# howardlau1999/pytorch-ddp-template

Hardware: NVIDIA H100
Metric: samples/sec (whole box, device-timed, max over ranks) for ResNet-50 DDP at 1/2/4/8 H100 (higher is better)
Workload: dtype bf16; 1 GPU; model=resnet50, global_batch=32, per_gpu_batch=32, image_size=224, parallelism=dp1, loss=mse(dense one-hot target), optimizer=sgd lr1e-3 + clip_grad_norm 1000 + linear warmup/decay, transport=single, cuda_graph=True

## Files before the change

b200ddp/csrc/batchnorm.cu:

```cuda
#include "ops.h"
#include "drv.h"
#include "tc_primitives.cuh"

#include <algorithm>
#include <cstdlib>
#include <map>
#include <mutex>
#include <utility>

namespace b200 {
namespace {

constexpr int kBnThreads = 256;
constexpr int kVec = 8;

template <typename T> __device__ __forceinline__ void bn_load8(const T* p, float* f);
template <> __device__ __forceinline__ void bn_load8<__nv_bfloat16>(const __nv_bfloat16* p, float* f) {
  unpack8(*reinterpret_cast<const Bf16x8*>(p), f);
}
template <> __device__ __forceinline__ void bn_load8<float>(const float* p, float* f) {
  const float4 a = reinterpret_cast<const float4*>(p)[0], b = reinterpret_cast<const float4*>(p)[1];
  f[0] = a.x; f[1] = a.y; f[2] = a.z; f[3] = a.w; f[4] = b.x; f[5] = b.y; f[6] = b.z; f[7] = b.w;
}
template <typename T> __device__ __forceinline__ void bn_store8(T* p, const float* f);
// ... 439 lines not shown
  const int cv = blockIdx.x * cvb + tx;
  if (cv * kVec >= C) return;
  const int S = gridDim.y;
  const int rows_per = (R + S - 1) / S;
  const int r0 = blockIdx.y * rows_per, r1 = min(R, r0 + rows_per);
  bn_bwd_apply_rows<T>(dy, x, y, dx, dres, save_mean, save_rstd, gamma, coef, C, cv, r0, r1, tyi, ty, relu);
}

template <typename T>
__global__ void __launch_bounds__(kBnThreads) bn_bwd_apply_pdl_kernel(const T* __restrict__ dy, const T* __restrict__ x, const unsigned char* __restrict__ y,
                                                                     T* __restrict__ dx, T* __restrict__ dres, const float* __restrict__ save_mean,
                                                                     const float* __restrict__ save_rstd, const float* __restrict__ gamma,
                                                                     const float* __restrict__ coef, int R, int C, int cvb, int ty, int relu) {
  const int tx = threadIdx.x % cvb, tyi = threadIdx.x / cvb;
  const int cv = blockIdx.x * cvb + tx;
  const int S = gridDim.y;
  const int rows_per = (R + S - 1) / S;
  const int r0 = blockIdx.y * rows_per, r1 = min(R, r0 + rows_per);
  bn_wait_producer();
  if (cv * kVec >= C) return;
  bn_bwd_apply_rows<T>(dy, x, y, dx, dres, save_mean, save_rstd, gamma, coef, C, cv, r0, r1, tyi, ty, relu);
}

int g_bn_pdl = -1;
bool bn_pdl_enabled() {
  if (g_bn_pdl < 0) { const char* e = getenv("B200DDP_PDL"); g_bn_pdl = (e && atoi(e) != 0) ? 1 : 0; }
  return g_bn_pdl > 0;
}

template <typename... KArgs, typename... Args>
void launch_dependent(void (*kernel)(KArgs...), dim3 grid, cudaStream_t s, Args... args) {
  cudaLaunchConfig_t cfg = {};
  cfg.gridDim = grid;
  cfg.blockDim = dim3(kBnThreads);
  cfg.dynamicSmemBytes = 0;
  cfg.stream = s;
  cudaLaunchAttribute attr[1];
  attr[0].id = cudaLaunchAttributeProgrammaticStreamSerialization;
  attr[0].val.programmaticStreamSerializationAllowed = 1;
  cfg.attrs = attr;
  cfg.numAttrs = 1;
  B200_CUDA_CHECK(cudaLaunchKernelEx(&cfg, kernel, static_cast<KArgs>(args)...));
}

Tile pick_tile(int R, int C) {
  Tile t;
  const int cv = C / kVec;
  t.cvb = cv < 8 ? cv : 8;
  while (kBnThreads % t.cvb != 0) --t.cvb;
  t.ty = kBnThreads / t.cvb;
  t.grid_x = (cv + t.cvb - 1) / t.cvb;
  int want = (4 * kNumSMs + t.grid_x - 1) / t.grid_x;
  int max_by_rows = R / (t.ty * 4);
  if (max_by_rows < 1) max_by_rows = 1;
  t.grid_y = want < max_by_rows ? want : max_by_rows;
  if (t.grid_y > 256) t.grid_y = 256;
  return t;
}

dim3 apply_grid(const Tile& t, int R) {
  int want = (8 * kNumSMs + t.grid_x - 1) / t.grid_x;
  int max_by_rows = R / (t.ty * 4);
  if (max_by_rows < 1) max_by_rows = 1;
  int gy = want < max_by_rows ? want : max_by_rows;
  return dim3(t.grid_x, gy);
}

bool fused_tile(int R, int C, Tile* t) {
  static int enabled = -1;
  if (enabled < 0) { const char* e = getenv("B200DDP_BN_FUSED"); enabled = (e && atoi(e) == 1) ? 1 : 0; }
  *t = pick_tile(R, C);
  if (!enabled || t->grid_x > 2 * kNumSMs) return false;
  int cap = (2 * kNumSMs) / t->grid_x;
  if (cap < 1) cap = 1;
  if (t->grid_y > cap) t->grid_y = cap;
  return true;
}

constexpr int kResThreads = 256;
constexpr int kResTile = 64;
constexpr int kResMaxBox = 256;
constexpr int kResMaxBoxes = 16;
constexpr int kResWarps = kResThreads / 32;
constexpr int kResMaxWaves = 2;
constexpr int kResFixedSmem = kResMaxBoxes * 8 + (kResWarps * 2 + 2 + 3) * kResTile * 4;

__device__ unsigned int g_bn_resident_error = 0;

struct ResGeom {
  int R, C;
  int T;
  int P;
  int box_rows;
  int nbox;
  int waves;
};

__device__ __forceinline__ void res_grid_sync(unsigned int* bar, unsigned int nblocks) {
  __syncthreads();
  if (threadIdx.x == 0) {
    unsigned int* gen = bar + 1;
    const unsigned int g0 = bn_ld_acquire(gen);
    __threadfence();
    if (atomicAdd(bar, 1u) == nblocks - 1) {
      atomicExch(bar, 0u);
      __threadfence();
      bn_st_release(gen, g0 + 1u);
    } else {
      unsigned long long t0;
      asm volatile("mov.u64 %0, %%globaltimer;" : "=l"(t0));
      while (bn_ld_acquire(gen) == g0) {
        unsigned long long t;
        asm volatile("mov.u64 %0, %%globaltimer;" : "=l"(t));
        if (t - t0 > 2000000000ull) { atomicExch(&g_bn_resident_error, 1u); break; }
      }
    }
    __threadfence();
  }
  __syncthreads();
}

__device__ __forceinline__ void res_write_partials(float (&acc)[2][kVec], float* red, float* __restrict__ partial, int P, int p, int C,
                                                   int c0) {
  const int lane = threadIdx.x & 31, warp = threadIdx.x >> 5, cv = threadIdx.x & 7;
#pragma unroll
  for (int a = 0; a < 2; ++a)
#pragma unroll
    for (int i = 0; i < kVec; ++i) {
      float v = acc[a][i];
      v += __shfl_xor_sync(0xffffffffu, v, 8);
      v += __shfl_xor_sync(0xffffffffu, v, 16);
      if (lane < 8) red[(warp * 2 + a) * kResTile + cv * kVec + i] = v;
    }
  __syncthreads();
  if (threadIdx.x < 2 * kResTile) {
    const int a = threadIdx.x / kResTile, c = threadIdx.x % kResTile;
    float s = 0.f;
    for (int w = 0; w < kResWarps; ++w) s += red[(w * 2 + a) * kResTile + c];
    if (c0 + c < C) partial[((size_t)a * P + p) * C + c0 + c] = s;
  }
}

__device__ __forceinline__ void res_reduce_partials(float* red, const float* __restrict__ partial, int P, int C, int c0) {
  const int q = threadIdx.x & 31, l = threadIdx.x >> 5;
  const int a = q >> 4, c4 = (q & 15) * 4;
  float4 s = make_float4(0.f, 0.f, 0.f, 0.f);
  if (c0 + c4 < C) {
    const float* base = partial + (size_t)a * P * C + c0 + c4;
#pragma unroll 4
    for (int k = l; k < P; k += kResWarps) {
      const float4 v = __ldcg(reinterpret_cast<const float4*>(base + (size_t)k * C));
      s.x += v.x; s.y += v.y; s.z += v.z; s.w += v.w;
    }
  }
  __syncthreads();
  *reinterpret_cast<float4*>(red + (l * 2 + a) * kResTile + c4) = s;
  __syncthreads();
  if (threadIdx.x < 2 * kResTile) {
    const int aa = threadIdx.x / kResTile, c = threadIdx.x % kResTile;
    float t = 0.f;
    for (int w = 0; w < kResWarps; ++w) t += red[(w * 2 + aa) * kResTile + c];
    red[kResWarps * 2 * kResTile + aa * kResTile + c] = t;
  }
  __syncthreads();
}

__device__ __forceinline__ void res_ld8(const unsigned char* s, float* f) { unpack8(*reinterpret_cast<const Bf16x8*>(s), f); }
__device__ __forceinline__ void res_st8(unsigned char* s, const float* f) { *reinterpret_cast<Bf16x8*>(s) = pack8(f); }

__global__ void __launch_bounds__(kResThreads, 2)
bn_resident_fwd_kernel(const __grid_constant__ CUtensorMap map_x, const __grid_constant__ CUtensorMap map_y,
                       const __grid_constant__ CUtensorMap map_res, const __nv_bfloat16* __restrict__ residual, unsigned char* __restrict__ mask, const float* __restrict__ gamma,
                       const float* __restrict__ beta, float* __restrict__ running_mean, float* __restrict__ running_var,
                       long long* __restrict__ num_batches, float* __restrict__ save_mean, float* __restrict__ save_rstd,
                       float* __restrict__ scale, float* __restrict__ shift, float* __restrict__ partial, unsigned int* __restrict__ bar,
                       float eps, float momentum, int relu, const ResGeom g) {
  extern __shared__ __align__(128) unsigned char res_smem[];
  const int slab_rows = g.nbox * g.box_rows;
  const uint32_t box_bytes = (uint32_t)g.box_rows * kResTile * 2;
  unsigned char* data = res_smem;
  uint64_t* mbar = reinterpret_cast<uint64_t*>(res_smem + (size_t)slab_rows * kResTile * 2);
  float* red = reinterpret_cast<float*>(mbar + kResMaxBoxes);
  float* coef = red + kResWarps * 2 * kResTile + 2 * kResTile;
  const int cv = threadIdx.x & 7, rl = threadIdx.x >> 3;
  const int ntiles = (g.C + kResTile - 1) / kResTile, cvs = g.C / kVec;
  const int slot = blockIdx.x / g.P, p = blockIdx.x % g.P;
  const int r0 = p * slab_rows;
  const int nlive = r0 >= g.R ? 0 : min(g.nbox, (g.R - r0 + g.box_rows - 1) / g.box_rows);
  if (threadIdx.x == 0) {
    for (int b = 0; b < g.nbox; ++b) tc::mbar_init(&mbar[b], 1);
    asm volatile("fence.mbarrier_init.release.cluster;" ::: "memory");
    tc::tma_prefetch_desc(&map_x);
    tc::tma_prefetch_desc(&map_y);
    if (blockIdx.x == 0 && num_batches != nullptr) *num_batches += 1;
  }
  __syncthreads();
  for (int w = 0; w < g.waves; ++w) {
    const int t = w * g.T + slot;
    const bool active = t < ntiles;
    const int c0 = t * kResTile;
    const int cvg = t * (kResTile / kVec) + cv;
    if (active && threadIdx.x == 0) {
      for (int b = 0; b < nlive; ++b) {
        tc::mbar_expect_tx(&mbar[b], box_bytes);
        tc::tma_load_2d(&map_x, &mbar[b], data + (size_t)b * box_bytes, c0, r0 + b * g.box_rows);
      }
    }
    float acc[2][kVec];
#pragma unroll
    for (int i = 0; i < kVec; ++i) { acc[0][i] = 0.f; acc[1][i] = 0.f; }
    if (active) {
      for (int b = 0; b < nlive; ++b) {
        tc::mbar_wait(&mbar[b], (uint32_t)(w & 1));
        const unsigned char* box = data + (size_t)b * box_bytes + cv * 16;
        for (int rr = rl; rr < g.box_rows; rr += 4 * 32) {
          float f[4][kVec];
#pragma unroll
          for (int u = 0; u < 4; ++u) {
            if (rr + u * 32 < g.box_rows) res_ld8(box + (size_t)(rr + u * 32) * (kResTile * 2), f[u]);
            else
#pragma unroll
              for (int i = 0; i < kVec; ++i) f[u][i] = 0.f;
          }
#pragma unroll
          for (int u = 0; u < 4; ++u)
#pragma unroll
            for (int i = 0; i < kVec; ++i) { acc[0][i] += f[u][i]; acc[1][i] = fmaf(f[u][i], f[u][i], acc[1][i]); }
        }
      }
      if (residual != nullptr && threadIdx.x == 0) {
        for (int b = 0; b < nlive; ++b)
          asm volatile("cp.async.bulk.prefetch.tensor.2d.L2.global [%0, {%1, %2}];"
                       ::"l"(reinterpret_cast<uint64_t>(&map_res)), "r"(c0), "r"(r0 + b * g.box_rows) : "memory");
      }
      res_write_partials(acc, red, partial, g.P, p, g.C, c0);
    }
    res_grid_sync(bar, gridDim.x);
    if (!active) continue;
    res_reduce_partials(red, partial, g.P, g.C, c0);
    if (threadIdx.x < kResTile) {
      const float* tot = red + kResWarps * 2 * kResTile;
      const int c = threadIdx.x, ch = c0 + c;
      if (ch < g.C) {
        const float inv_r = 1.f / (float)g.R;
        const float mean = tot[c] * inv_r;
        const float var = fmaxf(tot[kResTile + c] * inv_r - mean * mean, 0.f);
        const float rstd = rsqrtf(var + eps);
        const float sc = gamma[ch] * rstd;
        const float sh = beta[ch] - mean * sc;
        coef[c] = sc;
        coef[kResTile + c] = sh;
        if (p == 0) {
          save_mean[ch] = mean;
          save_rstd[ch] = rstd;
          scale[ch] = sc;
          shift[ch] = sh;
          if (running_mean != nullptr) {
            const float unbiased = g.R > 1 ? var * ((float)g.R / (float)(g.R - 1)) : var;
            running_mean[ch] = (1.f - momentum) * running_mean[ch] + momentum * mean;
            running_var[ch] = (1.f - momentum) * running_var[ch] + momentum * unbiased;
          }
        }
      } else {
        coef[c] = 0.f;
        coef[kResTile + c] = 0.f;
      }
    }
    __syncthreads();
    float sc[kVec], sh[kVec];
#pragma unroll
    for (int i = 0; i < kVec; ++i) { sc[i] = coef[cv * kVec + i]; sh[i] = coef[kResTile + cv * kVec + i]; }
    const bool live_cv = cvg < cvs;
    for (int b = 0; b < nlive; ++b) {
      unsigned char* box = data + (size_t)b * box_bytes + cv * 16;
      const int rb = r0 + b * g.box_rows;
      for (int rr = rl; rr < g.box_rows; rr += 8 * 32) {
        Bf16x8 rv[8];
#pragma unroll
        for (int u = 0; u < 8; ++u) {
          const int r = rb + rr + u * 32;
          if (residual != nullptr && rr + u * 32 < g.box_rows && r < g.R && live_cv)
            rv[u] = *reinterpret_cast<const Bf16x8*>(residual + (size_t)r * g.C + (size_t)cvg * kVec);
        }
#pragma unroll
        for (int u = 0; u < 8; ++u) {
          const int r = rb + rr + u * 32;
          if (!(rr + u * 32 < g.box_rows && r < g.R && live_cv)) continue;
          float f[kVec], rs[kVec];
          res_ld8(box + (size_t)(rr + u * 32) * (kResTile * 2), f);
          if (residual != nullptr) unpack8(rv[u], rs);
          unsigned int bits = 0;
#pragma unroll
          for (int i = 0; i < kVec; ++i) {
            float v = fmaf(f[i], sc[i], sh[i]);
            if (residual != nullptr) v += rs[i];
            bits |= (v > 0.f ? 1u : 0u) << i;
            f[i] = relu ? fmaxf(v, 0.f) : v;
          }
          res_st8(box + (size_t)(rr + u * 32) * (kResTile * 2), f);
          if (mask != nullptr) mask[(size_t)r * cvs + cvg] = (unsigned char)bits;
        }
      }
      tc::fence_async_smem();
      __syncthreads();
      if (threadIdx.x == 0) { tc::tma_store_2d(&map_y, data + (size_t)b * box_bytes, c0, rb); tc::bulk_commit(); }
    }
    if (threadIdx.x == 0) asm volatile("cp.async.bulk.wait_group.read 0;" ::: "memory");
    __syncthreads();
  }
  if (threadIdx.x == 0) tc::bulk_wait_all();
}

__global__ void __launch_bounds__(kResThreads, 2)
bn_resident_bwd_kernel(const __grid_constant__ CUtensorMap map_dy, const __grid_constant__ CUtensorMap map_x,
                       const __grid_constant__ CUtensorMap map_dx, const __grid_constant__ CUtensorMap map_dres,
                       const unsigned char* __restrict__ mask, const float* __restrict__ save_mean, const float* __restrict__ save_rstd,
                       const float* __restrict__ gamma, float* __restrict__ dgamma, float* __restrict__ dbeta, float* __restrict__ coef_out,
                       float* __restrict__ partial, unsigned int* __restrict__ bar, int relu, int want_dres, const ResGeom g) {
  extern __shared__ __align__(128) unsigned char res_smem[];
  const int slab_rows = g.nbox * g.box_rows;
  const uint32_t box_bytes = (uint32_t)g.box_rows * kResTile * 2;
  unsigned char* dyd = res_smem;
  unsigned char* xd = res_smem + (size_t)slab_rows * kResTile * 2;
  uint64_t* mbar = reinterpret_cast<uint64_t*>(res_smem + (size_t)2 * slab_rows * kResTile * 2);
  float* red = reinterpret_cast<float*>(mbar + kResMaxBoxes);
  float* coef = red + kResWarps * 2 * kResTile + 2 * kResTile;
  unsigned char* smask = reinterpret_cast<unsigned char*>(coef + 3 * kResTile);
  const int cv = threadIdx.x & 7, rl = threadIdx.x >> 3;
  const int ntiles = (g.C + kResTile - 1) / kResTile, cvs = g.C / kVec;
  const int slot = blockIdx.x / g.P, p = blockIdx.x % g.P;
  const int r0 = p * slab_rows;
  const int nlive = r0 >= g.R ? 0 : min(g.nbox, (g.R - r0 + g.box_rows - 1) / g.box_rows);
  if (threadIdx.x == 0) {
    for (int b = 0; b < g.nbox; ++b) tc::mbar_init(&mbar[b], 1);
    asm volatile("fence.mbarrier_init.release.cluster;" ::: "memory");
    tc::tma_prefetch_desc(&map_dy);
    tc::tma_prefetch_desc(&map_x);
  }
  __syncthreads();
  for (int w = 0; w < g.waves; ++w) {
    const int t = w * g.T + slot;
    const bool active = t < ntiles;
    const int c0 = t * kResTile;
    const int cvg = t * (kResTile / kVec) + cv;
    const bool live_cv = cvg < cvs;
    if (active && threadIdx.x == 0) {
      for (int b = 0; b < nlive; ++b) {
        tc::mbar_expect_tx(&mbar[b], 2 * box_bytes);
        tc::tma_load_2d(&map_dy, &mbar[b], dyd + (size_t)b * box_bytes, c0, r0 + b * g.box_rows);
        tc::tma_load_2d(&map_x, &mbar[b], xd + (size_t)b * box_bytes, c0, r0 + b * g.box_rows);
      }
    }
    if (active && relu) {
      const int n = min(slab_rows, g.R - r0) * 8;
#pragma unroll 8
      for (int i = threadIdx.x; i < n; i += kResThreads) {
        const int cg = t * (kResTile / kVec) + (i & 7);
        smask[i] = cg < cvs ? mask[(size_t)(r0 + (i >> 3)) * cvs + cg] : 0u;
      }
      __syncthreads();
    }
    float acc[2][kVec];
#pragma unroll
    for (int i = 0; i < kVec; ++i) { acc[0][i] = 0.f; acc[1][i] = 0.f; }
    if (active) {
      float mean[kVec], rstd[kVec];
#pragma unroll
      for (int i = 0; i < kVec; ++i) { mean[i] = 0.f; rstd[i] = 0.f; }
      if (live_cv) { bn_load8<float>(save_mean + cvg * kVec, mean); bn_load8<float>(save_rstd + cvg * kVec, rstd); }
      for (int b = 0; b < nlive; ++b) {
        tc::mbar_wait(&mbar[b], (uint32_t)(w & 1));
        for (int rr = rl; rr < g.box_rows; rr += 2 * 32) {
          float gv[2][kVec], xv[2][kVec];
          unsigned int mk[2];
#pragma unroll
          for (int u = 0; u < 2; ++u) {
            const int q = min(rr + u * 32, g.box_rows - 1);
            res_ld8(dyd + (size_t)b * box_bytes + (size_t)q * (kResTile * 2) + cv * 16, gv[u]);
            res_ld8(xd + (size_t)b * box_bytes + (size_t)q * (kResTile * 2) + cv * 16, xv[u]);
            mk[u] = rr + u * 32 < g.box_rows ? (relu ? smask[(b * g.box_rows + q) * 8 + cv] : 0xffu) : 0u;
          }
#pragma unroll
          for (int u = 0; u < 2; ++u)
#pragma unroll
            for (int i = 0; i < kVec; ++i) {
              const float gm = ((mk[u] >> i) & 1u) ? gv[u][i] : 0.f;
              acc[0][i] += gm;
              acc[1][i] = fmaf(gm, (xv[u][i] - mean[i]) * rstd[i], acc[1][i]);
            }
        }
      }
      res_write_partials(acc, red, partial, g.P, p, g.C, c0);
    }
    res_grid_sync(bar, gridDim.x);
    if (!active) continue;
    res_reduce_partials(red, partial, g.P, g.C, c0);
    if (threadIdx.x < kResTile) {
      const float* tot = red + kResWarps * 2 * kResTile;
      const int c = threadIdx.x, ch = c0 + c;
      float ka = 0.f, kb = 0.f, kc = 0.f;
      if (ch < g.C) {
        const float inv_r = 1.f / (float)g.R;
        const float s1 = tot[c], s2 = tot[kResTile + c];
        const float c1 = s1 * inv_r, c2 = s2 * inv_r;
        const float mean = save_mean[ch], rstd = save_rstd[ch];
        ka = gamma[ch] * rstd;
        kb = -ka * rstd * c2;
        kc = -ka * (c1 - mean * rstd * c2);
        if (p == 0) {
          dbeta[ch] = s1;
          dgamma[ch] = s2;
          coef_out[ch] = c1;
          coef_out[g.C + ch] = c2;
        }
      }
      coef[c] = ka;
      coef[kResTile + c] = kb;
      coef[2 * kResTile + c] = kc;
    }
    __syncthreads();
    float ka[kVec], kb[kVec], kc[kVec];
#pragma unroll
    for (int i = 0; i < kVec; ++i) {
      ka[i] = coef[cv * kVec + i];
      kb[i] = coef[kResTile + cv * kVec + i];
      kc[i] = coef[2 * kResTile + cv * kVec + i];
    }
    for (int b = 0; b < nlive; ++b) {
      const int rb = r0 + b * g.box_rows;
      unsigned char* gbox = dyd + (size_t)b * box_bytes + cv * 16;
      unsigned char* xbox = xd + (size_t)b * box_bytes + cv * 16;
      for (int rr = rl; rr < g.box_rows; rr += 2 * 32) {
        float gv[2][kVec], xv[2][kVec];
        unsigned int mk[2];
#pragma unroll
        for (int u = 0; u < 2; ++u) {
          const int q = min(rr + u * 32, g.box_rows - 1);
          res_ld8(gbox + (size_t)q * (kResTile * 2), gv[u]);
          res_ld8(xbox + (size_t)q * (kResTile * 2), xv[u]);
          mk[u] = relu ? smask[(b * g.box_rows + q) * 8 + cv] : 0xffu;
        }
#pragma unroll
        for (int u = 0; u < 2; ++u) {
          if (rr + u * 32 >= g.box_rows) continue;
          const size_t off = (size_t)(rr + u * 32) * (kResTile * 2);
          float o[kVec];
#pragma unroll
          for (int i = 0; i < kVec; ++i) {
            if (!((mk[u] >> i) & 1u)) gv[u][i] = 0.f;
            o[i] = fmaf(ka[i], gv[u][i], fmaf(kb[i], xv[u][i], kc[i]));
          }
          if (want_dres) res_st8(gbox + off, gv[u]);
          res_st8(xbox + off, o);
        }
      }
      tc::fence_async_smem();
      __syncthreads();
      if (threadIdx.x == 0) {
        tc::tma_store_2d(&map_dx, xd + (size_t)b * box_bytes, c0, rb);
        if (want_dres) tc::tma_store_2d(&map_dres, dyd + (size_t)b * box_bytes, c0, rb);
        tc::bulk_commit();
      }
    }
    if (threadIdx.x == 0) asm volatile("cp.async.bulk.wait_group.read 0;" ::: "memory");
    __syncthreads();
  }
  if (threadIdx.x == 0) tc::bulk_wait_all();
}

int g_bn_two_pass = 0;

bool resident_allowed() {
  static int fused_env = -1;
  if (fused_env < 0) { const char* e = getenv("B200DDP_BN_FUSED"); fused_env = (e && atoi(e) == 1) ? 1 : 0; }
  return !g_bn_two_pass && !fused_env && !bn_pdl_enabled();
}

struct ResPlan {
  bool ok = false;
  ResGeom g{};
  int grid = 0;
  int smem = 0;
};

ResPlan resident_plan(int R, int C, int streams) {
  static std::mutex mu;
  static std::map<std::pair<int, std::pair<long long, int>>, ResPlan> cache;
  int dev = 0;
  B200_CUDA_CHECK(cudaGetDevice(&dev));
  const auto key = std::make_pair(dev, std::make_pair(((long long)R << 20) | (long long)C, streams));
  std::lock_guard<std::mutex> lock(mu);
  auto it = cache.find(key);
  if (it != cache.end()) return it->second;
  ResPlan plan;
  int sms = 0, optin = 0;
  B200_CUDA_CHECK(cudaDeviceGetAttribute(&sms, cudaDevAttrMultiProcessorCount, dev));
  B200_CUDA_CHECK(cudaDeviceGetAttribute(&optin, cudaDevAttrMaxSharedMemoryPerBlockOptin, dev));
  const long long budget = (long long)optin - kResFixedSmem - 1024;
  const int ntiles = (C + kResTile - 1) / kResTile;
  const long long row_bytes = (long long)kResTile * 2 * streams + (streams == 2 ? 8 : 0);
  for (int T = ntiles; T >= 1 && R > 0; --T) {
    int P = sms / T;
    if (P < 1) continue;
    P = std::min(P, std::max(1, (R + 31) / 32));
    const int need = (R + P - 1) / P;
    const int nbox = (need + kResMaxBox - 1) / kResMaxBox;
    if (nbox > kResMaxBoxes) continue;
    const int box_rows = (need + nbox - 1) / nbox;
    const long long slab = (long long)nbox * box_rows * row_bytes;
    if (slab > budget) continue;
    if ((ntiles + T - 1) / T > kResMaxWaves) break;
    plan.g = ResGeom{R, C, T, (R + nbox * box_rows - 1) / (nbox * box_rows), box_rows, nbox, (ntiles + T - 1) / T};
    plan.grid = plan.g.T * plan.g.P;
    plan.smem = (int)slab + kResFixedSmem;
    plan.ok = true;
    break;
  }
  cache.emplace(key, plan);
  return plan;
}

CUtensorMap res_map(const void* ptr, int R, int C, int box_rows) {
  auto& drv = Driver::get();
  if (!drv.TensorMapEncodeTiled) throw std::runtime_error("batch norm: cuTensorMapEncodeTiled unavailable");
  CUtensorMap map;
  cuuint64_t dims[2] = {(cuuint64_t)C, (cuuint64_t)R};
  cuuint64_t strides[1] = {(cuuint64_t)C * 2};
  cuuint32_t box[2] = {(cuuint32_t)kResTile, (cuuint32_t)box_rows};
  cuuint32_t es[2] = {1, 1};
  B200_DRV_CHECK(drv.TensorMapEncodeTiled(&map, CU_TENSOR_MAP_DATA_TYPE_BFLOAT16, 2, const_cast<void*>(ptr), dims, strides, box, es,
                                          CU_TENSOR_MAP_INTERLEAVE_NONE, CU_TENSOR_MAP_SWIZZLE_NONE, CU_TENSOR_MAP_L2_PROMOTION_L2_256B,
                                          CU_TENSOR_MAP_FLOAT_OOB_FILL_NONE));
  return map;
}

int res_smem_limit() {
  int dev = 0, optin = 0;
  B200_CUDA_CHECK(cudaGetDevice(&dev));
  B200_CUDA_CHECK(cudaDeviceGetAttribute(&optin, cudaDevAttrMaxSharedMemoryPerBlockOptin, dev));
  return optin;
}

bool res_aligned(const void* p) { return p == nullptr || (reinterpret_cast<uintptr_t>(p) & 15u) == 0; }

template <typename... KArgs, typename... Args>
void launch_cooperative(void (*kernel)(KArgs...), const ResPlan& plan, cudaStream_t s, Args... args) {
  cudaLaunchConfig_t cfg = {};
  cfg.gridDim = dim3(plan.grid);
  cfg.blockDim = dim3(kResThreads);
  cfg.dynamicSmemBytes = plan.smem;
  cfg.stream = s;
  cudaLaunchAttribute attr[1];
  attr[0].id = cudaLaunchAttributeCooperative;
  attr[0].val.cooperative = 1;
  cfg.attrs = attr;
  cfg.numAttrs = 1;
  B200_CUDA_CHECK(cudaLaunchKernelEx(&cfg, kernel, static_cast<KArgs>(args)...));
}

}

template <typename T>
__global__ void __launch_bounds__(kBnThreads) bn_apply_partials_kernel(const T* __restrict__ x, const T* __restrict__ residual, T* __restrict__ y,
                                                                      unsigned char* __restrict__ mask, const float* __restrict__ partial, int G,
                                                                      const float* __restrict__ gamma, const float* __restrict__ beta,
                                                                      float* __restrict__ running_mean, float* __restrict__ running_var,
                                                                      long long* __restrict__ num_batches, float* __restrict__ save_mean,
                                                                      float* __restrict__ save_rstd, float eps, float momentum, int R, int C,
                                                                      int cvb, int ty, int relu) {
  extern __shared__ float bn_smem[];
  const int tx = threadIdx.x % cvb, tyi = threadIdx.x / cvb;
  const int cv = blockIdx.x * cvb + tx;
  const bool live = cv * kVec < C;
  float acc[2][kVec];
#pragma unroll
  for (int i = 0; i < kVec; ++i) { acc[0][i] = 0.f; acc[1][i] = 0.f; }
  if (live) {
    for (int g = tyi; g < G; g += ty) {
      float a[kVec], b[kVec];
      bn_load8<float>(partial + (size_t)g * C + cv * kVec, a);
      bn_load8<float>(partial + ((size_t)G + g) * C + cv * kVec, b);
#pragma unroll
      for (int i = 0; i < kVec; ++i) { acc[0][i] += a[i]; acc[1][i] += b[i]; }
    }
  }
  reduce_rows<2>(acc, bn_smem, tx, tyi, cvb, ty);
  const int width = cvb * kVec;
  float* sc_s = bn_smem + 2 * ty * width;
  float* sh_s = sc_s + width;
  if (tyi == 0 && live) {
    const float inv_r = 1.f / (float)R;
#pragma unroll
    for (int i = 0; i < kVec; ++i) {
      const int ch = cv * kVec + i;
      const float sum = bn_smem[tx * kVec + i], sq = bn_smem[ty * width + tx * kVec + i];
      const float mean = sum * inv_r;
      const float var = fmaxf(sq * inv_r - mean * mean, 0.f);
      const float rstd = rsqrtf(var + eps);
      const float sc = gamma[ch] * rstd;
      sc_s[tx * kVec + i] = sc;
      sh_s[tx * kVec + i] = beta[ch] - mean * sc;
      if (blockIdx.y == 0) {
        save_mean[ch] = mean;
        save_rstd[ch] = rstd;
        if (running_mean != nullptr) {
          const float unbiased = R > 1 ? var * ((float)R / (float)(R - 1)) : var;
          running_mean[ch] = (1.f - momentum) * running_mean[ch] + momentum * mean;
          running_var[ch] = (1.f - momentum) * running_var[ch] + momentum * unbiased;
        }
      }
    }
  }
  if (blockIdx.x == 0 && blockIdx.y == 0 && threadIdx.x == 0 && num_batches != nullptr) *num_batches += 1;
  __syncthreads();
  if (!live) return;
  const int S = gridDim.y;
  const int rows_per = (R + S - 1) / S;
  const int r0 = blockIdx.y * rows_per, r1 = min(R, r0 + rows_per);
  bn_apply_rows<T>(x, residual, y, mask, sc_s - (size_t)blockIdx.x * width, sh_s - (size_t)blockIdx.x * width, C, cv, r0, r1, tyi, ty, relu);
}

template <typename T>
__global__ void __launch_bounds__(kBnThreads) bn_bwd_apply_partials_kernel(const T* __restrict__ dy, const T* __restrict__ x, const unsigned char* __restrict__ y,
                                                                          T* __restrict__ dx, T* __restrict__ dres, const float* __restrict__ partial, int G,
                                                                          const float* __restrict__ save_mean, const float* __restrict__ save_rstd,
                                                                          const float* __restrict__ gamma, float* __restrict__ dgamma,
                                                                          float* __restrict__ dbeta, int R, int C, int cvb, int ty, int relu) {
  extern __shared__ float bn_smem[];
  const int tx = threadIdx.x % cvb, tyi = threadIdx.x / cvb;
  const int cv = blockIdx.x * cvb + tx;
  const bool live = cv * kVec < C;
  float acc[2][kVec];
#pragma unroll
  for (int i = 0; i < kVec; ++i) { acc[0][i] = 0.f; acc[1][i] = 0.f; }
  if (live) {
    for (int g = tyi; g < G; g += ty) {
      float a[kVec], b[kVec];
      bn_load8<float>(partial + (size_t)g * C + cv * kVec, a);
      bn_load8<float>(partial + ((size_t)G + g) * C + cv * kVec, b);
#pragma unroll
      for (int i = 0; i < kVec; ++i) { acc[0][i] += a[i]; acc[1][i] += b[i]; }
    }
  }
  reduce_rows<2>(acc, bn_smem, tx, tyi, cvb, ty);
  const int width = cvb * kVec;
  float* c1_s = bn_smem + 2 * ty * width;
  float* c2_s = c1_s + width;
  if (tyi == 0 && live) {
    const float inv_r = 1.f / (float)R;
#pragma unroll
    for (int i = 0; i < kVec; ++i) {
      const int ch = cv * kVec + i;
      const float s1 = bn_smem[tx * kVec + i], s2 = bn_smem[ty * width + tx * kVec + i];
      c1_s[tx * kVec + i] = s1 * inv_r;
      c2_s[tx * kVec + i] = s2 * inv_r;
      if (blockIdx.y == 0) { dgamma[ch] = s2; dbeta[ch] = s1; }
    }
  }
  __syncthreads();
  if (!live) return;
  const int S = gridDim.y;
  const int rows_per = (R + S - 1) / S;
  const int r0 = blockIdx.y * rows_per, r1 = min(R, r0 + rows_per);
  bn_bwd_apply_rows_coef<T>(dy, x, y, dx, dres, save_mean, save_rstd, gamma, c1_s + tx * kVec, c2_s + tx * kVec, C, cv, r0, r1, tyi, ty, relu);
}

void set_bn_pdl(int on) { g_bn_pdl = on; }

void set_bn_two_pass(int on) { g_bn_two_pass = on ? 1 : 0; }

unsigned int bn_resident_error() {
  unsigned int v = 0;
  B200_CUDA_CHECK(cudaMemcpyFromSymbol(&v, g_bn_resident_error, sizeof(v)));
  return v;
}

void bn_workspace_sizes(int R, int C, size_t* partial_floats, size_t* counters) {
  const Tile t = pick_tile(R, C);
  const ResPlan fwd = resident_plan(R, C, 1), bwd = resident_plan(R, C, 2);
  const int p = std::max(fwd.ok ? fwd.g.P : 0, bwd.ok ? bwd.g.P : 0);
  *partial_floats = (size_t)2 * std::max(t.grid_y, p) * C;
  *counters = (size_t)2 * t.grid_x + 2;
}

void launch_bn_forward(const void* x, const void* residual, void* y, unsigned char* mask, DType dt, int R, int C, const float* gamma, const float* beta,
                       float* running_mean, float* running_var, long long* num_batches, float* save_mean, float* save_rstd,
                       float* scale, float* shift, float* partial, unsigned int* counters, float eps, float momentum, bool relu,
                       cudaStream_t s) {
  if (C % kVec != 0) throw std::runtime_error("fused batch norm: channel count must be a multiple of 8");
  const int r = relu ? 1 : 0;
  if (dt == DType::BF16 && resident_allowed() && res_aligned(x) && res_aligned(residual) && res_aligned(y)) {
    const ResPlan plan = resident_plan(R, C, 1);
    if (plan.ok) {
      static std::atomic<unsigned long long> smem_done{0};
      ensure_max_dynamic_smem(bn_resident_fwd_kernel, res_smem_limit(), smem_done);
      const CUtensorMap mx = res_map(x, R, C, plan.g.box_rows), my = res_map(y, R, C, plan.g.box_rows);
      const CUtensorMap mres = residual != nullptr ? res_map(residual, R, C, plan.g.box_rows) : mx;
      launch_cooperative(bn_resident_fwd_kernel, plan, s, mx, my, mres, (const __nv_bfloat16*)residual, mask, gamma, beta, running_mean, running_var,
                         num_batches, save_mean, save_rstd, scale, shift, partial, counters + 2 * pick_tile(R, C).grid_x, eps, momentum, r,
                         plan.g);
      B200_COUNT_LAUNCH(1);
      return;
    }
  }
  Tile t;
  const bool fused = fused_tile(R, C, &t);
  const size_t smem = (size_t)2 * t.ty * t.cvb * kVec * sizeof(float);
  const dim3 grid(t.grid_x, t.grid_y);
  if (!fused && bn_pdl_enabled()) {
#define B200_BN_FWD_PDL(T)                                                                                                                  \
    bn_stats_kernel<T, false, true><<<grid, kBnThreads, smem, s>>>((const T*)x, R, C, t.cvb, t.ty, partial, counters, gamma, beta, running_mean, \
                                                                   running_var, num_batches, save_mean, save_rstd, scale, shift, eps, momentum,  \
                                                                   (const T*)residual, (T*)y, mask, r);                                          \
    B200_CUDA_CHECK(cudaGetLastError()); B200_COUNT_LAUNCH(1);                                                                                   \
    launch_dependent(bn_apply_pdl_kernel<T>, apply_grid(t, R), s, (const T*)x, (const T*)residual, (T*)y, mask, (const float*)scale,              \
                     (const float*)shift, R, C, t.cvb, t.ty, r);                                                                                  \
    B200_COUNT_LAUNCH(1)
    if (dt == DType::BF16) { B200_BN_FWD_PDL(__nv_bfloat16); } else { B200_BN_FWD_PDL(float); }
#undef B200_BN_FWD_PDL
    return;
  }
#define B200_BN_FWD(T, F)                                                                                                            \
  bn_stats_kernel<T, F><<<grid, kBnThreads, smem, s>>>((const T*)x, R, C, t.cvb, t.ty, partial, counters, gamma, beta, running_mean, \
                                                       running_var, num_batches, save_mean, save_rstd, scale, shift, eps, momentum, \
                                                       (const T*)residual, (T*)y, mask, r)
  if (dt == DType::BF16) { if (fused) B200_BN_FWD(__nv_bfloat16, true); else B200_BN_FWD(__nv_bfloat16, false); }
  else { if (fused) B200_BN_FWD(float, true); else B200_BN_FWD(float, false); }
#undef B200_BN_FWD
  B200_CUDA_CHECK(cudaGetLastError()); B200_COUNT_LAUNCH(1);
  if (fused) return;
  if (dt == DType::BF16)
    bn_apply_kernel<__nv_bfloat16><<<apply_grid(t, R), kBnThreads, 0, s>>>((const __nv_bfloat16*)x, (const __nv_bfloat16*)residual,
                                                                           (__nv_bfloat16*)y, mask, scale, shift, R, C, t.cvb, t.ty, r);
  else
    bn_apply_kernel<float><<<apply_grid(t, R), kBnThreads, 0, s>>>((const float*)x, (const float*)residual, (float*)y, mask, scale, shift, R, C,
                                                                   t.cvb, t.ty, r);
  B200_CUDA_CHECK(cudaGetLastError()); B200_COUNT_LAUNCH(1);
}

void launch_bn_forward_from_partials(const void* x, const void* residual, void* y, unsigned char* mask, DType dt, int R, int C,
                                     const float* gamma, const float* beta, float* running_mean, float* running_var,
                                     long long* num_batches, float* save_mean, float* save_rstd, float* scale, float* shift,
                                     const float* partial, int groups, float eps, float momentum, bool relu, cudaStream_t s) {
  (void)scale; (void)shift;
  if (C % kVec != 0) throw std::runtime_error("fused batch norm: channel count must be a multiple of 8");
  if (groups < 1) throw std::runtime_error("fused batch norm: empty partial statistics");
  const Tile t = pick_tile(R, C);
  const int r = relu ? 1 : 0;
  const size_t smem = (size_t)(2 * t.ty + 2) * t.cvb * kVec * sizeof(float);
  if (dt == DType::BF16)
    bn_apply_partials_kernel<__nv_bfloat16><<<apply_grid(t, R), kBnThreads, smem, s>>>(
        (const __nv_bfloat16*)x, (const __nv_bfloat16*)residual, (__nv_bfloat16*)y, mask, partial, groups, gamma, beta, running_mean, running_var,
        num_batches, save_mean, save_rstd, eps, momentum, R, C, t.cvb, t.ty, r);
  else
    bn_apply_partials_kernel<float><<<apply_grid(t, R), kBnThreads, smem, s>>>(
        (const float*)x, (const float*)residual, (float*)y, mask, partial, groups, gamma, beta, running_mean, running_var, num_batches, save_mean,
        save_rstd, eps, momentum, R, C, t.cvb, t.ty, r);
  B200_CUDA_CHECK(cudaGetLastError()); B200_COUNT_LAUNCH(1);
}

void launch_bn_backward_from_partials(const void* dy, const void* x, const void* y, void* dx, void* dres, DType dt, int R, int C, const float* gamma,
                                      const float* save_mean, const float* save_rstd, float* dgamma, float* dbeta, const float* partial, int groups,
                                      bool relu, cudaStream_t s) {
  if (C % kVec != 0) throw std::runtime_error("fused batch norm: channel count must be a multiple of 8");
  if (groups < 1) throw std::runtime_error("fused batch norm: empty partial sums");
  const Tile t = pick_tile(R, C);
  const int r = relu ? 1 : 0;
  const size_t smem = (size_t)(2 * t.ty + 2) * t.cvb * kVec * sizeof(float);
  if (dt == DType::BF16)
    bn_bwd_apply_partials_kernel<__nv_bfloat16><<<apply_grid(t, R), kBnThreads, smem, s>>>(
        (const __nv_bfloat16*)dy, (const __nv_bfloat16*)x, (const unsigned char*)y, (__nv_bfloat16*)dx, (__nv_bfloat16*)dres, partial, groups, save_mean,
        save_rstd, gamma, dgamma, dbeta, R, C, t.cvb, t.ty, r);
  else
    bn_bwd_apply_partials_kernel<float><<<apply_grid(t, R), kBnThreads, smem, s>>>(
        (const float*)dy, (const float*)x, (const unsigned char*)y, (float*)dx, (float*)dres, partial, groups, save_mean, save_rstd, gamma, dgamma, dbeta,
        R, C, t.cvb, t.ty, r);
  B200_CUDA_CHECK(cudaGetLastError()); B200_COUNT_LAUNCH(1);
}

void launch_bn_backward(const void* dy, const void* x, const void* y, void* dx, void* dres, DType dt, int R, int C, const float* gamma,
                        const float* save_mean, const float* save_rstd, float* dgamma, float* dbeta, float* coef, float* partial,
                        unsigned int* counters, bool relu, cudaStream_t s) {
  if (C % kVec != 0) throw std::runtime_error("fused batch norm: channel count must be a multiple of 8");
  const int r = relu ? 1 : 0;
  if (dt == DType::BF16 && resident_allowed() && res_aligned(dy) && res_aligned(x) && res_aligned(dx) && res_aligned(dres)) {
    const ResPlan plan = resident_plan(R, C, 2);
    if (plan.ok) {
      static std::atomic<unsigned long long> smem_done{0};
      ensure_max_dynamic_smem(bn_resident_bwd_kernel, res_smem_limit(), smem_done);
      const int br = plan.g.box_rows;
      const CUtensorMap mdy = res_map(dy, R, C, br), mx = res_map(x, R, C, br), mdx = res_map(dx, R, C, br);
      const CUtensorMap mdres = dres != nullptr ? res_map(dres, R, C, br) : mdx;
      launch_cooperative(bn_resident_bwd_kernel, plan, s, mdy, mx, mdx, mdres, (const unsigned char*)y, save_mean, save_rstd, gamma, dgamma,
                         dbeta, coef, partial, counters + 2 * pick_tile(R, C).grid_x, r, dres != nullptr ? 1 : 0, plan.g);
      B200_COUNT_LAUNCH(1);
      return;
    }
  }
  Tile t;
  const bool fused = fused_tile(R, C, &t);
  const size_t smem = (size_t)2 * t.ty * t.cvb * kVec * sizeof(float);
  const dim3 grid(t.grid_x, t.grid_y);
  if (!fused && bn_pdl_enabled()) {
#define B200_BN_BWD_PDL(T)                                                                                                                   \
    bn_bwd_reduce_kernel<T, false, true><<<grid, kBnThreads, smem, s>>>((const T*)dy, (const T*)x, (const unsigned char*)y, R, C, t.cvb, t.ty, r,  \
                                                                        save_mean, save_rstd, partial, counters, dgamma, dbeta, coef, gamma,      \
                                                                        (T*)dx, (T*)dres);                                                        \
    B200_CUDA_CHECK(cudaGetLastError()); B200_COUNT_LAUNCH(1);                                                                                     \
    launch_dependent(bn_bwd_apply_pdl_kernel<T>, apply_grid(t, R), s, (const T*)dy, (const T*)x, (const unsigned char*)y, (T*)dx, (T*)dres,         \
                     save_mean, save_rstd, gamma, (const float*)coef, R, C, t.cvb, t.ty, r);                                                        \
    B200_COUNT_LAUNCH(1)
    if (dt == DType::BF16) { B200_BN_BWD_PDL(__nv_bfloat16); } else { B200_BN_BWD_PDL(float); }
#undef B200_BN_BWD_PDL
    return;
  }
#define B200_BN_BWD(T, F)                                                                                                              \
  bn_bwd_reduce_kernel<T, F><<<grid, kBnThreads, smem, s>>>((const T*)dy, (const T*)x, (const unsigned char*)y, R, C, t.cvb, t.ty, r,  \
                                                            save_mean, save_rstd, partial, counters, dgamma, dbeta, coef, gamma,      \
                                                            (T*)dx, (T*)dres)
  if (dt == DType::BF16) { if (fused) B200_BN_BWD(__nv_bfloat16, true); else B200_BN_BWD(__nv_bfloat16, false); }
  else { if (fused) B200_BN_BWD(float, true); else B200_BN_BWD(float, false); }
#undef B200_BN_BWD
  B200_CUDA_CHECK(cudaGetLastError()); B200_COUNT_LAUNCH(1);
  if (fused) return;
  if (dt == DType::BF16)
    bn_bwd_apply_kernel<__nv_bfloat16><<<apply_grid(t, R), kBnThreads, 0, s>>>((const __nv_bfloat16*)dy, (const __nv_bfloat16*)x, (const unsigned char*)y,
                                                                               (__nv_bfloat16*)dx, (__nv_bfloat16*)dres, save_mean, save_rstd, gamma, coef,
                                                                               R, C, t.cvb, t.ty, r);
  else
    bn_bwd_apply_kernel<float><<<apply_grid(t, R), kBnThreads, 0, s>>>((const float*)dy, (const float*)x, (const unsigned char*)y, (float*)dx,
                                                                       (float*)dres, save_mean, save_rstd, gamma, coef, R, C, t.cvb, t.ty, r);
  B200_CUDA_CHECK(cudaGetLastError()); B200_COUNT_LAUNCH(1);
}

}
```

Baseline: 4952 samples/s.

## Pipeline resident batchnorm tiles with per-tile barriers and multi-launch splitting

Reworks the SMEM-resident batchnorm forward and backward kernels. Each channel tile now syncs only its own group of P blocks through acq_rel atomics instead of doing a full grid barrier with threadfences. The next tile's TMA loads are issued as soon as each box's store has drained, and residual and parameter loads are prefetched before the barrier. The partial-sum reduction is unrolled with a P cap, mask loads are vectorised, and large channel counts are split across multiple cooperative launches, dropping occupancy to 1 block/SM. The aim is to hide barrier and load latency and to let more layers use the resident path, at the cost of extra launches, more registers, and more counters.

```diff
diff --git a/b200ddp/csrc/batchnorm.cu b/b200ddp/csrc/batchnorm.cu
--- a/b200ddp/csrc/batchnorm.cu
+++ b/b200ddp/csrc/batchnorm.cu
@@ -545,7 +545,10 @@
 constexpr int kResMaxBox = 256;
 constexpr int kResMaxBoxes = 16;
 constexpr int kResWarps = kResThreads / 32;
+static_assert(kResMaxBox <= 8 * (kResThreads / 8), "the forward apply gives each of the 32 row lanes 8 rows of a box");
 constexpr int kResMaxWaves = 2;
+constexpr int kResMaxLaunches = 2;
+constexpr int kResMaxPartialLoads = 17;
 constexpr int kResFixedSmem = kResMaxBoxes * 8 + (kResWarps * 2 + 2 + 3) * kResTile * 4;
 
 __device__ unsigned int g_bn_resident_error = 0;
@@ -557,17 +560,19 @@
   int box_rows;
   int nbox;
   int waves;
+  int tile0;
+  int tile_end;
 };
 
-__device__ __forceinline__ void res_grid_sync(unsigned int* bar, unsigned int nblocks) {
+__device__ __forceinline__ void res_tile_sync(unsigned int* bar, unsigned int nblocks) {
   __syncthreads();
   if (threadIdx.x == 0) {
     unsigned int* gen = bar + 1;
     const unsigned int g0 = bn_ld_acquire(gen);
-    __threadfence();
-    if (atomicAdd(bar, 1u) == nblocks - 1) {
-      atomicExch(bar, 0u);
-      __threadfence();
+    unsigned int old;
+    asm volatile("atom.add.acq_rel.gpu.global.u32 %0, [%1], 1;" : "=r"(old) : "l"(bar) : "memory");
+    if (old == nblocks - 1) {
+      asm volatile("st.relaxed.gpu.global.u32 [%0], 0;" ::"l"(bar) : "memory");
       bn_st_release(gen, g0 + 1u);
     } else {
       unsigned long long t0;
@@ -578,7 +583,6 @@
         if (t - t0 > 2000000000ull) { atomicExch(&g_bn_resident_error, 1u); break; }
       }
     }
-    __threadfence();
   }
   __syncthreads();
 }
@@ -610,11 +614,13 @@
   float4 s = make_float4(0.f, 0.f, 0.f, 0.f);
   if (c0 + c4 < C) {
     const float* base = partial + (size_t)a * P * C + c0 + c4;
-#pragma unroll 4
-    for (int k = l; k < P; k += kResWarps) {
-      const float4 v = __ldcg(reinterpret_cast<const float4*>(base + (size_t)k * C));
-      s.x += v.x; s.y += v.y; s.z += v.z; s.w += v.w;
-    }
+    float4 v[kResMaxPartialLoads];
+#pragma unroll
+    for (int j = 0; j < kResMaxPartialLoads; ++j)
+      if (l + j * kResWarps < P) v[j] = __ldcg(reinterpret_cast<const float4*>(base + (size_t)(l + j * kResWarps) * C));
+#pragma unroll
+    for (int j = 0; j < kResMaxPartialLoads; ++j)
+      if (l + j * kResWarps < P) { s.x += v[j].x; s.y += v[j].y; s.z += v[j].z; s.w += v[j].w; }
   }
   __syncthreads();
   *reinterpret_cast<float4*>(red + (l * 2 + a) * kResTile + c4) = s;
@@ -631,7 +637,7 @@
 __device__ __forceinline__ void res_ld8(const unsigned char* s, float* f) { unpack8(*reinterpret_cast<const Bf16x8*>(s), f); }
 __device__ __forceinline__ void res_st8(unsigned char* s, const float* f) { *reinterpret_cast<Bf16x8*>(s) = pack8(f); }
 
-__global__ void __launch_bounds__(kResThreads, 2)
+__global__ void __launch_bounds__(kResThreads, 1)
 bn_resident_fwd_kernel(const __grid_constant__ CUtensorMap map_x, const __grid_constant__ CUtensorMap map_y,
                        const __grid_constant__ CUtensorMap map_res, const __nv_bfloat16* __restrict__ residual, unsigned char* __restrict__ mask, const float* __restrict__ gamma,
                        const float* __restrict__ beta, float* __restrict__ running_mean, float* __restrict__ running_var,
@@ -646,33 +652,42 @@
   float* red = reinterpret_cast<float*>(mbar + kResMaxBoxes);
   float* coef = red + kResWarps * 2 * kResTile + 2 * kResTile;
   const int cv = threadIdx.x & 7, rl = threadIdx.x >> 3;
-  const int ntiles = (g.C + kResTile - 1) / kResTile, cvs = g.C / kVec;
+  const int cvs = g.C / kVec;
   const int slot = blockIdx.x / g.P, p = blockIdx.x % g.P;
   const int r0 = p * slab_rows;
   const int nlive = r0 >= g.R ? 0 : min(g.nbox, (g.R - r0 + g.box_rows - 1) / g.box_rows);
+  bar += 2 * slot;
+  auto load_box = [&](int b, int t) {
+    tc::mbar_expect_tx(&mbar[b], box_bytes);
+    tc::tma_load_2d(&map_x, &mbar[b], data + (size_t)b * box_bytes, t * kResTile, r0 + b * g.box_rows);
+  };
   if (threadIdx.x == 0) {
     for (int b = 0; b < g.nbox; ++b) tc::mbar_init(&mbar[b], 1);
     asm volatile("fence.mbarrier_init.release.cluster;" ::: "memory");
     tc::tma_prefetch_desc(&map_x);
     tc::tma_prefetch_desc(&map_y);
-    if (blockIdx.x == 0 && num_batches != nullptr) *num_batches += 1;
+    if (blockIdx.x == 0 && g.tile0 == 0 && num_batches != nullptr) *num_batches += 1;
+    if (g.tile0 + slot < g.tile_end)
+      for (int b = 0; b < nlive; ++b) load_box(b, g.tile0 + slot);
   }
   __syncthreads();
   for (int w = 0; w < g.waves; ++w) {
-    const int t = w * g.T + slot;
-    const bool active = t < ntiles;
+    const int t = g.tile0 + w * g.T + slot;
+    if (t >= g.tile_end) break;
+    const bool next = t + g.T < g.tile_end;
     const int c0 = t * kResTile;
     const int cvg = t * (kResTile / kVec) + cv;
-    if (active && threadIdx.x == 0) {
-      for (int b = 0; b < nlive; ++b) {
-        tc::mbar_expect_tx(&mbar[b], box_bytes);
-        tc::tma_load_2d(&map_x, &mbar[b], data + (size_t)b * box_bytes, c0, r0 + b * g.box_rows);
-      }
+    float gm = 0.f, bt = 0.f, rmean = 0.f, rvar = 0.f;
+    if (threadIdx.x < kResTile && c0 + (int)threadIdx.x < g.C) {
+      const int ch = c0 + threadIdx.x;
+      gm = gamma[ch];
+      bt = beta[ch];
+      if (p == 0 && running_mean != nullptr) { rmean = running_mean[ch]; rvar = running_var[ch]; }
     }
     float acc[2][kVec];
 #pragma unroll
     for (int i = 0; i < kVec; ++i) { acc[0][i] = 0.f; acc[1][i] = 0.f; }
-    if (active) {
+    {
       for (int b = 0; b < nlive; ++b) {
         tc::mbar_wait(&mbar[b], (uint32_t)(w & 1));
         const unsigned char* box = data + (size_t)b * box_bytes + cv * 16;
@@ -698,8 +713,18 @@
       }
       res_write_partials(acc, red, partial, g.P, p, g.C, c0);
     }
-    res_grid_sync(bar, gridDim.x);
-    if (!active) continue;
+    const bool live_cv = cvg < cvs;
+    auto load_res = [&](int b, Bf16x8 (&d)[8]) {
+#pragma unroll
+      for (int u = 0; u < 8; ++u) {
+        const int q = rl + u * 32, r = r0 + b * g.box_rows + q;
+        if (residual != nullptr && q < g.box_rows && r < g.R && live_cv)
+          d[u] = *reinterpret_cast<const Bf16x8*>(residual + (size_t)r * g.C + (size_t)cvg * kVec);
+      }
+    };
+    Bf16x8 rv[8];
+    if (nlive > 0) load_res(0, rv);
+    res_tile_sync(bar, g.P);
     res_reduce_partials(red, partial, g.P, g.C, c0);
     if (threadIdx.x < kResTile) {
       const float* tot = red + kResWarps * 2 * kResTile;
@@ -709,8 +734,8 @@
         const float mean = tot[c] * inv_r;
         const float var = fmaxf(tot[kResTile + c] * inv_r - mean * mean, 0.f);
         const float rstd = rsqrtf(var + eps);
-        const float sc = gamma[ch] * rstd;
-        const float sh = beta[ch] - mean * sc;
+        const float sc = gm * rstd;
+        const float sh = bt - mean * sc;
         coef[c] = sc;
         coef[kResTile + c] = sh;
         if (p == 0) {
@@ -720,8 +745,8 @@
           shift[ch] = sh;
           if (running_mean != nullptr) {
             const float unbiased = g.R > 1 ? var * ((float)g.R / (float)(g.R - 1)) : var;
-            running_mean[ch] = (1.f - momentum) * running_mean[ch] + momentum * mean;
-            running_var[ch] = (1.f - momentum) * running_var[ch] + momentum * unbiased;
+            running_mean[ch] = (1.f - momentum) * rmean + momentum * mean;
+            running_var[ch] = (1.f - momentum) * rvar + momentum * unbiased;
           }
         }
       } else {
@@ -733,48 +758,49 @@
     float sc[kVec], sh[kVec];
 #pragma unroll
     for (int i = 0; i < kVec; ++i) { sc[i] = coef[cv * kVec + i]; sh[i] = coef[kResTile + cv * kVec + i]; }
-    const bool live_cv = cvg < cvs;
     for (int b = 0; b < nlive; ++b) {
       unsigned char* box = data + (size_t)b * box_bytes + cv * 16;
       const int rb = r0 + b * g.box_rows;
-      for (int rr = rl; rr < g.box_rows; rr += 8 * 32) {
-        Bf16x8 rv[8];
-#pragma unroll
-        for (int u = 0; u < 8; ++u) {
-          const int r = rb + rr + u * 32;
-          if (residual != nullptr && rr + u * 32 < g.box_rows && r < g.R && live_cv)
-            rv[u] = *reinterpret_cast<const Bf16x8*>(residual + (size_t)r * g.C + (size_t)cvg * kVec);
+      Bf16x8 rn[8];
+      if (b + 1 < nlive) load_res(b + 1, rn);
+#pragma unroll
+      for (int u = 0; u < 8; ++u) {
+        const int q = rl + u * 32, r = rb + q;
+        if (!(q < g.box_rows && r < g.R && live_cv)) continue;
+        float f[kVec], rs[kVec];
+        res_ld8(box + (size_t)q * (kResTile * 2), f);
+        if (residual != nullptr) unpack8(rv[u], rs);
+        unsigned int bits = 0;
+#pragma unroll
+        for (int i = 0; i < kVec; ++i) {
+          float v = fmaf(f[i], sc[i], sh[i]);
+          if (residual != nullptr) v += rs[i];
+          bits |= (v > 0.f ? 1u : 0u) << i;
+          f[i] = relu ? fmaxf(v, 0.f) : v;
         }
-#pragma unroll
-        for (int u = 0; u < 8; ++u) {
-          const int r = rb + rr + u * 32;
-          if (!(rr + u * 32 < g.box_rows && r < g.R && live_cv)) continue;
-          float f[kVec], rs[kVec];
-          res_ld8(box + (size_t)(rr + u * 32) * (kResTile * 2), f);
-          if (residual != nullptr) unpack8(rv[u], rs);
-          unsigned int bits = 0;
-#pragma unroll
-          for (int i = 0; i < kVec; ++i) {
-            float v = fmaf(f[i], sc[i], sh[i]);
-            if (residual != nullptr) v += rs[i];
-            bits |= (v > 0.f ? 1u : 0u) << i;
-            f[i] = relu ? fmaxf(v, 0.f) : v;
-          }
-          res_st8(box + (size_t)(rr + u * 32) * (kResTile * 2), f);
-          if (mask != nullptr) mask[(size_t)r * cvs + cvg] = (unsigned char)bits;
-        }
-      }
+        res_st8(box + (size_t)q * (kResTile * 2), f);
+        if (mask != nullptr) mask[(size_t)r * cvs + cvg] = (unsigned char)bits;
+      }
+#pragma unroll
+      for (int u = 0; u < 8; ++u) rv[u] = rn[u];
       tc::fence_async_smem();
       __syncthreads();
-      if (threadIdx.x == 0) { tc::tma_store_2d(&map_y, data + (size_t)b * box_bytes, c0, rb); tc::bulk_commit(); }
-    }
-    if (threadIdx.x == 0) asm volatile("cp.async.bulk.wait_group.read 0;" ::: "memory");
+      if (threadIdx.x == 0) {
+        tc::tma_store_2d(&map_y, data + (size_t)b * box_bytes, c0, rb);
+        tc::bulk_commit();
+        if (next && b > 0) { asm volatile("cp.async.bulk.wait_group.read 1;" ::: "memory"); load_box(b - 1, t + g.T); }
+      }
+    }
+    if (threadIdx.x == 0) {
+      asm volatile("cp.async.bulk.wait_group.read 0;" ::: "memory");
+      if (next && nlive > 0) load_box(nlive - 1, t + g.T);
+    }
     __syncthreads();
   }
   if (threadIdx.x == 0) tc::bulk_wait_all();
 }
 
-__global__ void __launch_bounds__(kResThreads, 2)
+__global__ void __launch_bounds__(kResThreads, 1)
 bn_resident_bwd_kernel(const __grid_constant__ CUtensorMap map_dy, const __grid_constant__ CUtensorMap map_x,
                        const __grid_constant__ CUtensorMap map_dx, const __grid_constant__ CUtensorMap map_dres,
                        const unsigned char* __restrict__ mask, const float* __restrict__ save_mean, const float* __restrict__ save_rstd,
@@ -790,43 +816,60 @@
   float* coef = red + kResWarps * 2 * kResTile + 2 * kResTile;
   unsigned char* smask = reinterpret_cast<unsigned char*>(coef + 3 * kResTile);
   const int cv = threadIdx.x & 7, rl = threadIdx.x >> 3;
-  const int ntiles = (g.C + kResTile - 1) / kResTile, cvs = g.C / kVec;
+  const int cvs = g.C / kVec;
   const int slot = blockIdx.x / g.P, p = blockIdx.x % g.P;
   const int r0 = p * slab_rows;
   const int nlive = r0 >= g.R ? 0 : min(g.nbox, (g.R - r0 + g.box_rows - 1) / g.box_rows);
+  const bool mask_words = g.C % kResTile == 0 && (reinterpret_cast<uintptr_t>(mask) & 7u) == 0;
+  bar += 2 * slot;
+  auto load_box = [&](int b, int t) {
+    tc::mbar_expect_tx(&mbar[b], 2 * box_bytes);
+    tc::tma_load_2d(&map_dy, &mbar[b], dyd + (size_t)b * box_bytes, t * kResTile, r0 + b * g.box_rows);
+    tc::tma_load_2d(&map_x, &mbar[b], xd + (size_t)b * box_bytes, t * kResTile, r0 + b * g.box_rows);
+  };
   if (threadIdx.x == 0) {
     for (int b = 0; b < g.nbox; ++b) tc::mbar_init(&mbar[b], 1);
     asm volatile("fence.mbarrier_init.release.cluster;" ::: "memory");
     tc::tma_prefetch_desc(&map_dy);
     tc::tma_prefetch_desc(&map_x);
+    if (g.tile0 + slot < g.tile_end)
+      for (int b = 0; b < nlive; ++b) load_box(b, g.tile0 + slot);
   }
   __syncthreads();
   for (int w = 0; w < g.waves; ++w) {
-    const int t = w * g.T + slot;
-    const bool active = t < ntiles;
+    const int t = g.tile0 + w * g.T + slot;
+    if (t >= g.tile_end) break;
+    const bool next = t + g.T < g.tile_end;
     const int c0 = t * kResTile;
     const int cvg = t * (kResTile / kVec) + cv;
     const bool live_cv = cvg < cvs;
-    if (active && threadIdx.x == 0) {
-      for (int b = 0; b < nlive; ++b) {
-        tc::mbar_expect_tx(&mbar[b], 2 * box_bytes);
-        tc::tma_load_2d(&map_dy, &mbar[b], dyd + (size_t)b * box_bytes, c0, r0 + b * g.box_rows);
-        tc::tma_load_2d(&map_x, &mbar[b], xd + (size_t)b * box_bytes, c0, r0 + b * g.box_rows);
-      }
-    }
-    if (active && relu) {
-      const int n = min(slab_rows, g.R - r0) * 8;
+    float gam = 0.f, smean = 0.f, srstd = 0.f;
+    if (threadIdx.x < kResTile && c0 + (int)threadIdx.x < g.C) {
+      const int ch = c0 + threadIdx.x;
+      gam = gamma[ch];
+      smean = save_mean[ch];
+      srstd = save_rstd[ch];
+    }
+    if (relu) {
+      const int rows = min(slab_rows, g.R - r0);
+      if (mask_words) {
+#pragma unroll 4
+        for (int i = threadIdx.x; i < rows; i += kResThreads)
+          reinterpret_cast<unsigned long long*>(smask)[i] =
+              *reinterpret_cast<const unsigned long long*>(mask + (size_t)(r0 + i) * cvs + t * (kResTile / kVec));
+      } else {
 #pragma unroll 8
-      for (int i = threadIdx.x; i < n; i += kResThreads) {
-        const int cg = t * (kResTile / kVec) + (i & 7);
-        smask[i] = cg < cvs ? mask[(size_t)(r0 + (i >> 3)) * cvs + cg] : 0u;
+        for (int i = threadIdx.x; i < rows * 8; i += kResThreads) {
+          const int cg = t * (kResTile / kVec) + (i & 7);
+          smask[i] = cg < cvs ? mask[(size_t)(r0 + (i >> 3)) * cvs + cg] : 0u;
+        }
       }
       __syncthreads();
     }
     float acc[2][kVec];
 #pragma unroll
     for (int i = 0; i < kVec; ++i) { acc[0][i] = 0.f; acc[1][i] = 0.f; }
-    if (active) {
+    {
       float mean[kVec], rstd[kVec];
 #pragma unroll
       for (int i = 0; i < kVec; ++i) { mean[i] = 0.f; rstd[i] = 0.f; }
@@ -855,8 +898,7 @@
       }
       res_write_partials(acc, red, partial, g.P, p, g.C, c0);
     }
-    res_grid_sync(bar, gridDim.x);
-    if (!active) continue;
+    res_tile_sync(bar, g.P);
     res_reduce_partials(red, partial, g.P, g.C, c0);
     if (threadIdx.x < kResTile) {
       const float* tot = red + kResWarps * 2 * kResTile;
@@ -866,8 +908,8 @@
         const float inv_r = 1.f / (float)g.R;
         const float s1 = tot[c], s2 = tot[kResTile + c];
         const float c1 = s1 * inv_r, c2 = s2 * inv_r;
-        const float mean = save_mean[ch], rstd = save_rstd[ch];
-        ka = gamma[ch] * rstd;
+        const float mean = smean, rstd = srstd;
+        ka = gam * rstd;
         kb = -ka * rstd * c2;
         kc = -ka * (c1 - mean * rstd * c2);
         if (p == 0) {
@@ -923,9 +965,13 @@
         tc::tma_store_2d(&map_dx, xd + (size_t)b * box_bytes, c0, rb);
         if (want_dres) tc::tma_store_2d(&map_dres, dyd + (size_t)b * box_bytes, c0, rb);
         tc::bulk_commit();
-      }
-    }
-    if (threadIdx.x == 0) asm volatile("cp.async.bulk.wait_group.read 0;" ::: "memory");
+        if (next && b > 0) { asm volatile("cp.async.bulk.wait_group.read 1;" ::: "memory"); load_box(b - 1, t + g.T); }
+      }
+    }
+    if (threadIdx.x == 0) {
+      asm volatile("cp.async.bulk.wait_group.read 0;" ::: "memory");
+      if (next && nlive > 0) load_box(nlive - 1, t + g.T);
+    }
     __syncthreads();
   }
   if (threadIdx.x == 0) tc::bulk_wait_all();
@@ -942,6 +988,7 @@
 struct ResPlan {
   bool ok = false;
   ResGeom g{};
+  int launches = 0;
   int grid = 0;
   int smem = 0;
 };
@@ -963,7 +1010,7 @@
   const int ntiles = (C + kResTile - 1) / kResTile;
   const long long row_bytes = (long long)kResTile * 2 * streams + (streams == 2 ? 8 : 0);
   for (int T = ntiles; T >= 1 && R > 0; --T) {
-    int P = sms / T;
+    int P = std::min(sms / T, kResMaxPartialLoads * kResWarps);
     if (P < 1) continue;
     P = std::min(P, std::max(1, (R + 31) / 32));
     const int need = (R + P - 1) / P;
@@ -972,8 +1019,11 @@
     const int box_rows = (need + nbox - 1) / nbox;
     const long long slab = (long long)nbox * box_rows * row_bytes;
     if (slab > budget) continue;
-    if ((ntiles + T - 1) / T > kResMaxWaves) break;
-    plan.g = ResGeom{R, C, T, (R + nbox * box_rows - 1) / (nbox * box_rows), box_rows, nbox, (ntiles + T - 1) / T};
+    const int waves = (ntiles + T - 1) / T;
+    if (waves > kResMaxLaunches * kResMaxWaves) break;
+    plan.launches = (waves + kResMaxWaves - 1) / kResMaxWaves;
+    const int per_launch = (waves + plan.launches - 1) / plan.launches;
+    plan.g = ResGeom{R, C, T, (R + nbox * box_rows - 1) / (nbox * box_rows), box_rows, nbox, per_launch, 0, std::min(ntiles, T * per_launch)};
     plan.grid = plan.g.T * plan.g.P;
     plan.smem = (int)slab + kResFixedSmem;
     plan.ok = true;
@@ -981,6 +1031,13 @@
   }
   cache.emplace(key, plan);
   return plan;
+}
+
+ResGeom res_launch(const ResPlan& plan, int k) {
+  ResGeom g = plan.g;
+  g.tile0 = k * g.T * g.waves;
+  g.tile_end = std::min((g.C + kResTile - 1) / kResTile, g.tile0 + g.T * g.waves);
+  return g;
 }
 
 CUtensorMap res_map(const void* ptr, int R, int C, int box_rows) {
@@ -1143,7 +1200,7 @@
   const ResPlan fwd = resident_plan(R, C, 1), bwd = resident_plan(R, C, 2);
   const int p = std::max(fwd.ok ? fwd.g.P : 0, bwd.ok ? bwd.g.P : 0);
   *partial_floats = (size_t)2 * std::max(t.grid_y, p) * C;
-  *counters = (size_t)2 * t.grid_x + 2;
+  *counters = (size_t)2 * t.grid_x + 2 * (size_t)((C + kResTile - 1) / kResTile);
 }
 
 void launch_bn_forward(const void* x, const void* residual, void* y, unsigned char* mask, DType dt, int R, int C, const float* gamma, const float* beta,
@@ -1159,10 +1216,11 @@
       ensure_max_dynamic_smem(bn_resident_fwd_kernel, res_smem_limit(), smem_done);
       const CUtensorMap mx = res_map(x, R, C, plan.g.box_rows), my = res_map(y, R, C, plan.g.box_rows);
       const CUtensorMap mres = residual != nullptr ? res_map(residual, R, C, plan.g.box_rows) : mx;
-      launch_cooperative(bn_resident_fwd_kernel, plan, s, mx, my, mres, (const __nv_bfloat16*)residual, mask, gamma, beta, running_mean, running_var,
-                         num_batches, save_mean, save_rstd, scale, shift, partial, counters + 2 * pick_tile(R, C).grid_x, eps, momentum, r,
-                         plan.g);
-      B200_COUNT_LAUNCH(1);
+      for (int k = 0; k < plan.launches; ++k)
+        launch_cooperative(bn_resident_fwd_kernel, plan, s, mx, my, mres, (const __nv_bfloat16*)residual, mask, gamma, beta, running_mean,
+                           running_var, num_batches, save_mean, save_rstd, scale, shift, partial, counters + 2 * pick_tile(R, C).grid_x, eps,
+                           momentum, r, res_launch(plan, k));
+      B200_COUNT_LAUNCH(plan.launches);
       return;
     }
   }
@@ -1254,9 +1312,10 @@
       const int br = plan.g.box_rows;
       const CUtensorMap mdy = res_map(dy, R, C, br), mx = res_map(x, R, C, br), mdx = res_map(dx, R, C, br);
       const CUtensorMap mdres = dres != nullptr ? res_map(dres, R, C, br) : mdx;
-      launch_cooperative(bn_resident_bwd_kernel, plan, s, mdy, mx, mdx, mdres, (const unsigned char*)y, save_mean, save_rstd, gamma, dgamma,
-                         dbeta, coef, partial, counters + 2 * pick_tile(R, C).grid_x, r, dres != nullptr ? 1 : 0, plan.g);
-      B200_COUNT_LAUNCH(1);
+      for (int k = 0; k < plan.launches; ++k)
+        launch_cooperative(bn_resident_bwd_kernel, plan, s, mdy, mx, mdx, mdres, (const unsigned char*)y, save_mean, save_rstd, gamma, dgamma,
+                           dbeta, coef, partial, counters + 2 * pick_tile(R, C).grid_x, r, dres != nullptr ? 1 : 0, res_launch(plan, k));
+      B200_COUNT_LAUNCH(plan.launches);
       return;
     }
   }
```

Result: faster. 5140 samples/s (median of 6 runs) (+3.8%).
